# kakaobrain/hqtransformer

Measured on AMD Instinct MI355X. Metric: images/sec (256x256 class-cond sampling), higher is better.
Workload: dtype bf16

## Files before the change

hqtransformer_amd/csrc/common.h:

```cpp
#pragma once
#include <hip/hip_runtime.h>
#include <stdint.h>
#include <string>

typedef uint16_t bf16_t;

__device__ __host__ inline float bf16_to_f32(bf16_t v) {
    union { uint32_t u; float f; } c;
    c.u = ((uint32_t)v) << 16;
    return c.f;
}
__device__ __forceinline__ void bf16x8_to_f32(const uint4& raw, float (&f)[8]) {
    const unsigned w[4] = {raw.x, raw.y, raw.z, raw.w};
#pragma unroll
    for (int i = 0; i < 4; ++i) { f[2 * i] = bf16_to_f32((bf16_t)(w[i] & 0xffffu)); f[2 * i + 1] = bf16_to_f32((bf16_t)(w[i] >> 16)); }
}
__device__ __host__ inline bf16_t f32_to_bf16(float f) {
#if defined(__HIP_DEVICE_COMPILE__)
    return __builtin_bit_cast(bf16_t, (__bf16)f);
#endif
    union { uint32_t u; float f; } c;
    c.f = f;
    if ((c.u & 0x7fffffffu) > 0x7f800000u) return (bf16_t)((c.u >> 16) | 0x40);
    return (bf16_t)((c.u + 0x7fffu + ((c.u >> 16) & 1u)) >> 16);
}

enum { ACT_NONE = 0, ACT_GELU_ERF = 1, ACT_GELU_SIGMOID = 2 };
enum { STORE_ROWS = 0, STORE_NCHW = 1, STORE_QKV = 2, STORE_PACKED = 3, STORE_RESID = 4, STORE_ARGMIN = 5 };

__device__ __host__ inline int conv_ks(int taps) { return taps == 9 ? 3 : (taps == 16 ? 4 : 1); }
__device__ __host__ inline uint32_t float_order_key(float f) {
    union { float f; uint32_t u; } c;
    c.f = f;
    return (c.u & 0x80000000u) ? ~c.u : (c.u | 0x80000000u);
}

__device__ __host__ inline long long packed_off(int m, int k, int MB) {
    return ((long long)(k >> 4) * MB + (m >> 5)) * 512 + ((((k >> 3) & 1) << 5) + (m & 31)) * 8 + (k & 7);
}
constexpr int PACKED_MAX_ROWS = 16384;
__device__ __host__ inline int packed_mb(int M) {
    if (M > PACKED_MAX_ROWS) return 0;
    int mb = 1;
    while (mb * 32 < M) mb <<= 1;
    return mb;
}

struct ChainSync {
    const unsigned* wait;
    unsigned target;
    unsigned* signal;
    unsigned* err;
};

#define HQT_CHAIN_SPIN_LIMIT (1u << 17)
__device__ inline unsigned chain_poll(const ChainSync& c) {
    return c.wait ? __hip_atomic_load(c.wait, __ATOMIC_RELAXED, __HIP_MEMORY_SCOPE_AGENT) : 0u;
}
__device__ inline void chain_wait(const ChainSync& c, unsigned polled) {
    if (!c.wait) return;
    if (threadIdx.x == 0) {
        unsigned spins = 0;
        while (polled < c.target) {
            if (++spins > HQT_CHAIN_SPIN_LIMIT) { if (c.err) *c.err = 1u; break; }
            __builtin_amdgcn_s_sleep(1);
            polled = __hip_atomic_load(c.wait, __ATOMIC_RELAXED, __HIP_MEMORY_SCOPE_AGENT);
        }
        __builtin_amdgcn_fence(__ATOMIC_ACQUIRE, "agent");
        asm volatile("s_waitcnt vmcnt(0)" ::: "memory");
    }
    __syncthreads();
}
__device__ inline void chain_signal(const ChainSync& c) {
    if (!c.signal) return;
    asm volatile("s_waitcnt vmcnt(0)" ::: "memory");
    __syncthreads();
    if (threadIdx.x == 0) {
        __builtin_amdgcn_fence(__ATOMIC_RELEASE, "agent");
        asm volatile("s_waitcnt vmcnt(0)" ::: "memory");
        __hip_atomic_fetch_add(c.signal, 1u, __ATOMIC_RELAXED, __HIP_MEMORY_SCOPE_AGENT);
    }
}

struct GemmArgs {
    const void* A;
    int lda;
    long long a_batch_stride;
    int a_rows_per_group;
    int a_group_stride;
    int a_row_offset;
    int a_packed_mb;
    int conv_taps;
    int conv_stride2;
    int conv_nopad;
    int H, W, Cin;
    int upsample;
    const float* gn_stats;
    const float* gn_gamma;
    const float* gn_beta;
    int gn_groups;
    int gn_swish;
    const void* Bw;
    int ldb;
    long long b_batch_stride;
    void* C;
    int ldc;
    long long c_batch_stride;
    int M, N, K, batch;
    const float* bias;
    const void* resid;
    int act;
    float alpha;
    int store;
    int rows_per_group;
    int group_stride;
    int row_offset;
    const int* row_offset_dev;
    int rows_per_image;
    int clamp01;
    void* C2;
    void* C3;
    int qkv_D;
    int qkv_first;
    bf16_t* qkv_v_pk;
    int c_packed_mb;
    const void* zero_page;
    const float* ln_parts;
    int ln_nparts;
    const float* ln_colsum;
    float ln_eps;
    bf16_t* resid_pk;
    float* resid_parts;
    unsigned* tile_ctr;
    const float* am_rownorm;
    const float* am_colnorm;
    unsigned long long* am_best;
    ChainSync chain;
    float* gn_part_out;
    int gn_out_groups;
    int tune;
    const void* Bw_lo;
    const void* Bw_frag16;
    const void* Bw_up16;
    double* gn_part_out_d;
    int a_f32;
    int b_f32;
    int* range_flag;
    int out_split;
    int k_quarters;
    int b_tile16;
    int k_slices;
    float* k_slabs;
    int tile_panel;
    const int* row_pos;
};

__device__ __forceinline__ int row_live(const int* row_pos, int b) { const int p = row_pos[b]; return p < 0 ? 0 : p; }
__device__ __forceinline__ bool row_idle(const int* row_pos, int b) { return row_pos && row_pos[b] < 0; }
__device__ __forceinline__ int qkv_row_of(const GemmArgs& g, int b, int uniform) { return g.row_pos ? row_live(g.row_pos, b) : uniform; }

struct StepState {
    int step;
    int t_base;
};
__device__ __forceinline__ int step_of(const StepState* state, const int* row_pos, int b) { return row_pos ? row_live(row_pos, b) : state->step; }
struct RowKey {
    unsigned long long seed;
    long long global_row;
};
struct RowSampler {
    float temperature[3];
    int top_k[3];
    float top_p[3];
};
struct GuidePair {
    int pos_row, neg_row;
    float scale[3];
};

#define HQT_MAX_V 16384

__device__ __forceinline__ long long clamp_idx(long long v, int n) { return n > 0 ? (v < 0 ? 0 : (v >= n ? (long long)n - 1 : v)) : v; }
```

hqtransformer_amd/csrc/split_conv.hip:

```cpp
#include "split_kernels.h"
#include "split_ring.h"
#include "gemm_generic.h"
#include <algorithm>
#include <cstdlib>
#include <type_traits>

namespace {
__device__ __forceinline__ unsigned pack_h2(half_t a, half_t b) {
    return (unsigned)__builtin_bit_cast(unsigned short, a) | ((unsigned)__builtin_bit_cast(unsigned short, b) << 16);
}

__device__ __forceinline__ void xcd_tile(int& tile_m, int& tile_n) {
    const int nx = gridDim.x, total = gridDim.x * gridDim.y;
    int id = blockIdx.x + nx * blockIdx.y;
    if ((total & 7) == 0) id = (id & 7) * (total >> 3) + (id >> 3);
    tile_m = id / nx;
    tile_n = id - tile_m * nx;
}
}

__global__ void split_f32_kernel(const float* __restrict__ src, half_t* __restrict__ hi, half_t* __restrict__ lo, size_t n) {
    for (size_t i = blockIdx.x * (size_t)blockDim.x + threadIdx.x; i < n; i += (size_t)gridDim.x * blockDim.x) split2(src[i], hi[i], lo[i]);
}
hipError_t launch_split_f32(const float* src, half_t* hi, half_t* lo, size_t n, hipStream_t st) {
    split_f32_kernel<<<(int)std::min<size_t>((n + 255) / 256, 4096), 256, 0, st>>>(src, hi, lo, n);
    return hipGetLastError();
}

static inline int sp_chunk_pix(int HW) { int c = HW / 32; return c < 64 ? 64 : (c > 1024 ? 1024 : c); }
static inline bool sp_fixed_ok(int C) { return C % 8 == 0 && C / 8 <= 256 && 256 % (C / 8) == 0; }

#ifndef SP_INFLIGHT
#define SP_INFLIGHT 8
#endif
template <bool GN>
__global__ __launch_bounds__(256) void split_pack_kernel(const float* __restrict__ x, half_t* __restrict__ y, const float* __restrict__ stats,
                                                         const float* __restrict__ gamma, const float* __restrict__ beta, int HW, int C, int groups,
                                                         int swish, int nchunk, int chunk_pix, int* __restrict__ range_flag) {
    bool bad = false;
    const int b = blockIdx.x / nchunk, ch = blockIdx.x % nchunk;
    const int p0 = ch * chunk_pix, p1 = min(HW, p0 + chunk_pix);
    const int vpp = C / 8, rpi = 256 / vpp;
    const int cv = threadIdx.x % vpp, pl = threadIdx.x / vpp;
    float mu[8], rs[8], gm[8], bt[8];
    if (GN) {
        const int cpg = C / groups;
#pragma unroll
        for (int i = 0; i < 8; ++i) {
            const int c = cv * 8 + i;
            const float* st = stats + ((long long)b * groups + c / cpg) * 2;
            mu[i] = st[0]; rs[i] = st[1]; gm[i] = gamma[c]; bt[i] = beta[c];
        }
    }
    const float* xb = x + ((long long)b * HW) * C + cv * 8;
    half_t* yb = y + ((long long)b * HW) * 2 * C + cv * 8;
    auto emit = [&](const float4& a0, const float4& a1, int pix) {
        float f[8] = {a0.x, a0.y, a0.z, a0.w, a1.x, a1.y, a1.z, a1.w};
#pragma unroll
        for (int i = 0; i < 8; ++i) {
            if (GN) {
                float t = (f[i] - mu[i]) * rs[i] * gm[i] + bt[i];
                if (swish) t = t * __builtin_amdgcn_rcpf(1.0f + __expf(-t));
                f[i] = t;
            }
        }
        unsigned hi[4], lo[4];
        split8_checked(f, hi, lo, bad);
        const u32x4 vh = {hi[0], hi[1], hi[2], hi[3]};
        const u32x4 vl = {lo[0], lo[1], lo[2], lo[3]};
        half_t* dst = yb + (long long)pix * 2 * C;
        *reinterpret_cast<u32x4*>(dst) = vh;
        *reinterpret_cast<u32x4*>(dst + C) = vl;
    };
    int p = p0 + pl;
    constexpr int UF = SP_INFLIGHT;
    for (; p + (UF - 1) * rpi < p1; p += UF * rpi) {
        float4 r0[UF], r1[UF];
#pragma unroll
        for (int u = 0; u < UF; ++u) {
            const float* s = xb + (long long)(p + u * rpi) * C;
            r0[u] = *reinterpret_cast<const float4*>(s);
            r1[u] = *reinterpret_cast<const float4*>(s + 4);
        }
#pragma unroll
        for (int u = 0; u < UF; ++u) emit(r0[u], r1[u], p + u * rpi);
    }
    for (; p < p1; p += rpi) {
        const float* s = xb + (long long)p * C;
        emit(*reinterpret_cast<const float4*>(s), *reinterpret_cast<const float4*>(s + 4), p);
    }
    if (bad && range_flag) atomicOr(range_flag, 1);
}
__global__ __launch_bounds__(256) void split_pack_generic_kernel(const float* __restrict__ x, half_t* __restrict__ y, const float* __restrict__ stats,
                                                                 const float* __restrict__ gamma, const float* __restrict__ beta, long long total,
                                                                 int HW, int C, int groups, int swish, int* __restrict__ range_flag) {
    const int cpg = stats ? C / groups : 1;
    bool bad = false;
    for (long long i = blockIdx.x * (long long)blockDim.x + threadIdx.x; i < total; i += (long long)gridDim.x * blockDim.x) {
        const long long pix = i / C;
        const int c = (int)(i - pix * C);
        float t = x[i];
        if (stats) {
            const float* st = stats + ((pix / HW) * groups + c / cpg) * 2;
            t = (t - st[0]) * st[1] * gamma[c] + beta[c];
            if (swish) t = t / (1.0f + expf(-t));
        }
        half_t hi, lo;
        split2_checked(t, hi, lo, bad);
        y[pix * 2 * C + c] = hi;
        y[pix * 2 * C + C + c] = lo;
    }
    if (bad && range_flag) atomicOr(range_flag, 1);
}
hipError_t launch_split_pack(const float* x, half_t* y, const float* stats, const float* gamma, const float* beta, int B, int HW,
                             int C, int groups, int swish, int* range_flag, hipStream_t st) {
    if (sp_fixed_ok(C)) {
        const int cp = sp_chunk_pix(HW), nchunk = (HW + cp - 1) / cp;
        if (stats) split_pack_kernel<true><<<B * nchunk, 256, 0, st>>>(x, y, stats, gamma, beta, HW, C, groups, swish, nchunk, cp, range_flag);
        else split_pack_kernel<false><<<B * nchunk, 256, 0, st>>>(x, y, nullptr, nullptr, nullptr, HW, C, groups, 0, nchunk, cp, range_flag);
        return hipGetLastError();
    }
    const long long total = (long long)B * HW * C;
    split_pack_generic_kernel<<<(int)std::min<long long>((total + 255) / 256, 256 * 16), 256, 0, st>>>(x, y, stats, gamma, beta, total, HW, C, groups, swish, range_flag);
    return hipGetLastError();
}

namespace {
constexpr int S_TY = 8, S_TX = 16, S_PITCH = S_TX + 2;
constexpr int S_ROWS = (S_TY + 2) * S_PITCH;
constexpr int S_PIECES = (S_ROWS + 7) / 8;
constexpr int S_PATCH_BYTES = S_PIECES * 1024;
constexpr int S_CPITCH = R_CPITCH;
constexpr int split_conv3_lds(int BN) { return 4 * S_PATCH_BYTES + 4 * BN * 128; }
static_assert(128 * S_CPITCH <= split_conv3_lds(32), "epilogue staging must fit in the operand buffers");
static_assert(split_conv3_lds(128) <= 160 * 1024, "LDS budget");
}

template <bool NCHW, int BN, int PC = 0, int ABL = 0>
__global__ __launch_bounds__(PC ? 512 : 256, 1) void conv3x3_split_kernel(GemmArgs g) {
    static_assert(BN == 128 || (BN == 32 && NCHW), "the 32-channel variant exists for the NCHW conv_out store only");
    constexpr int WMW = BN == 128 ? 2 : 4, FJ = BN == 128 ? 2 : 1, B_BYTES = BN * 128;
    constexpr int FI = (S_TY / 2) / WMW;
    extern __shared__ __attribute__((aligned(16))) char lds_raw[];
    auto PATCH = [&](int s, int plane) -> char* { return lds_raw + (size_t)(s * 2 + plane) * S_PATCH_BYTES; };
    auto BT = [&](int s, int plane) -> char* { return lds_raw + 4 * S_PATCH_BYTES + (size_t)(s * 2 + plane) * B_BYTES; };
    const int tid = threadIdx.x & 255, lane = tid & 63, wave = tid >> 6;
    const bool producer = PC && threadIdx.x >= 256, consumer = !PC || threadIdx.x < 256;
    const int wm = BN == 128 ? wave >> 1 : wave, wn = BN == 128 ? wave & 1 : 0;
    const int fr = lane & 31, fh = lane >> 5;
    int tile_m, tile_n;
    xcd_tile(tile_m, tile_n);
    const int n0 = tile_n * BN;
    const int tiles_x = g.W / S_TX, tiles_y = g.H / S_TY;
    const int img = tile_m / (tiles_x * tiles_y);
    const int trem = tile_m - img * (tiles_x * tiles_y);
    const int ty0 = (trem / tiles_x) * S_TY, tx0 = (trem % tiles_x) * S_TX;
    const int Hin = g.H >> g.upsample, Win = g.W >> g.upsample;
    const half_t* Abase = reinterpret_cast<const half_t*>(g.A);
    const half_t* Bhi = reinterpret_cast<const half_t*>(g.Bw);
    const half_t* Blo = reinterpret_cast<const half_t*>(g.Bw_lo);
    const half_t* zero = reinterpret_cast<const half_t*>(g.zero_page);

    constexpr int PPW = (S_PIECES + 3) / 4;
    constexpr int BPW = BN / 32;
    long long boff[BPW];
#pragma unroll
    for (int i = 0; i < BPW; ++i) {
        const int row = (wave * BPW + i) * 8 + (lane >> 3);
        const int ch = ((lane & 7) ^ ((row >> 1) & 7)) * 8;
        boff[i] = (n0 + row < g.N) ? (long long)(n0 + row) * g.ldb + ch : -1;
    }
    auto issue_patch = [&](int c, int s) {
#pragma unroll
        for (int t = 0; t < PPW; ++t) {
            if (wave + 4 * t < S_PIECES) {
                const int q = (wave + 4 * t) * 8 + (lane >> 3);
                const int qy = (q * 3641) >> 16, qx = q - qy * S_PITCH;
                const int iy = ty0 + qy - 1, ix = tx0 + qx - 1;
                const int ch = ((lane & 7) ^ ((q >> 1) & 7)) * 8;
                const bool in = q < S_ROWS && (unsigned)iy < (unsigned)g.H && (unsigned)ix < (unsigned)g.W;
                const half_t* src = Abase + (((long long)img * Hin + (iy >> g.upsample)) * Win + (ix >> g.upsample)) * (2 * g.Cin) + ch + c * 64;
#pragma unroll
                for (int plane = 0; plane < 2; ++plane) {
                    const half_t* sp = in ? src + plane * g.Cin : zero;
                    char* dst = PATCH(s, plane) + (wave + 4 * t) * 1024;
                    __builtin_amdgcn_global_load_lds((const __attribute__((address_space(1))) void*)sp,
                                                     (__attribute__((address_space(3))) void*)dst, 16, 0, 0);
                }
            }
        }
    };
    auto issue_b = [&](int k0, int s) {
#pragma unroll
        for (int i = 0; i < BPW; ++i) {
            const half_t* sh = boff[i] >= 0 ? Bhi + boff[i] + k0 : zero;
            const half_t* sl = boff[i] >= 0 ? Blo + boff[i] + k0 : zero;
            char* dh = BT(s, 0) + (wave * BPW + i) * 1024;
            char* dl = BT(s, 1) + (wave * BPW + i) * 1024;
            __builtin_amdgcn_global_load_lds((const __attribute__((address_space(1))) void*)sh, (__attribute__((address_space(3))) void*)dh, 16, 0, 0);
            __builtin_amdgcn_global_load_lds((const __attribute__((address_space(1))) void*)sl, (__attribute__((address_space(3))) void*)dl, 16, 0, 0);
        }
    };

    f32x16 accm[FI][FJ], accx[FI][FJ];
#pragma unroll
    for (int i = 0; i < FI; ++i)
#pragma unroll
        for (int j = 0; j < FJ; ++j)
#pragma unroll
            for (int r = 0; r < 16; ++r) { accm[i][j][r] = 0.0f; accx[i][j][r] = 0.0f; }

    int qbase[FI];
#pragma unroll
    for (int i = 0; i < FI; ++i) qbase[i] = (wm * (2 * FI) + i * 2 + (fr >> 4)) * S_PITCH + (fr & 15);
    int brd[FJ];
#pragma unroll
    for (int j = 0; j < FJ; ++j) brd[j] = wn * 64 + j * 32 + fr;

    const unsigned lds_base = (unsigned)(size_t)(__attribute__((address_space(3))) char*)lds_raw;
    unsigned wa0[FJ];
#pragma unroll
    for (int j = 0; j < FJ; ++j) wa0[j] = brd[j] * 128 + ((fh ^ ((brd[j] >> 1) & 7)) << 4);
    auto compute = [&](int ps, int bs, int tapoff) {
        const unsigned pbase = lds_base + ps * 2 * S_PATCH_BYTES, wbase = lds_base + 4 * S_PATCH_BYTES + bs * 2 * B_BYTES;
        unsigned pa0[FI];
#pragma unroll
        for (int i = 0; i < FI; ++i) pa0[i] = (qbase[i] + tapoff) * 128 + ((fh ^ (((qbase[i] + tapoff) >> 1) & 7)) << 4);
        half8 ah[2][FI], al[2][FI], wh[2][FJ], wl[2][FJ];
        auto issue = [&](int ks, int set) {
#pragma unroll
            for (int j = 0; j < FJ; ++j) {
                const unsigned a = wbase + (wa0[j] ^ (ks << 5));
                asm volatile("ds_read_b128 %0, %1" : "=v"(wh[set][j]) : "v"(a));
                asm volatile("ds_read_b128 %0, %1 offset:%2" : "=v"(wl[set][j]) : "v"(a), "n"(B_BYTES));
            }
#pragma unroll
            for (int i = 0; i < FI; ++i) {
                const unsigned a = pbase + (pa0[i] ^ (ks << 5));
                asm volatile("ds_read_b128 %0, %1" : "=v"(ah[set][i]) : "v"(a));
                asm volatile("ds_read_b128 %0, %1 offset:%2" : "=v"(al[set][i]) : "v"(a), "n"(S_PATCH_BYTES));
            }
        };
#define HQT_RETIRE(set, P)                                                                                                          \
// ... 496 lines not shown
```

hqtransformer_amd/csrc/split_device.h:

```cpp
#pragma once
#include "split_kernels.h"

namespace {
constexpr float SPLIT_SCALE = 2048.0f, SPLIT_INV = 1.0f / 2048.0f;

__device__ __forceinline__ void split2(float x, half_t& hi, half_t& lo) {
    hi = (half_t)x;
    lo = (half_t)((x - (float)hi) * SPLIT_SCALE);
}
__device__ __forceinline__ void split2_checked(float x, half_t& hi, half_t& lo, bool& bad) {
    if (!(fabsf(x) < 65504.0f)) { bad = true; x = x > 0.0f ? 65472.0f : (x < 0.0f ? -65472.0f : 0.0f); }
    split2(x, hi, lo);
}
typedef float f32x2_t __attribute__((ext_vector_type(2)));
typedef _Float16 half2_t __attribute__((ext_vector_type(2)));
__device__ __forceinline__ void split8_checked(const float (&x)[8], unsigned (&hi)[4], unsigned (&lo)[4], bool& bad) {
#pragma unroll
    for (int p = 0; p < 4; ++p) {
        f32x2_t v = {x[2 * p], x[2 * p + 1]};
        bad |= !(fabsf(v.x) < 65504.0f) | !(fabsf(v.y) < 65504.0f);
        v.x = __builtin_amdgcn_fmed3f(v.x, -65472.0f, 65472.0f);
        v.y = __builtin_amdgcn_fmed3f(v.y, -65472.0f, 65472.0f);
        const half2_t h = __builtin_convertvector(v, half2_t);
        const f32x2_t r = (v - __builtin_convertvector(h, f32x2_t)) * SPLIT_SCALE;
        const half2_t l = __builtin_convertvector(r, half2_t);
        hi[p] = __builtin_bit_cast(unsigned, h);
        lo[p] = __builtin_bit_cast(unsigned, l);
    }
}
}
```

hqtransformer_amd/csrc/split_stream_conv.hip:

```cpp
#include "split_kernels.h"
#include "split_ring.h"
#include "gemm_generic.h"
#include "switches.h"
#include <algorithm>
#include <cstdlib>
#include <type_traits>

constexpr size_t R_FRAG_PAD = 3 * 4 * 512;
size_t split_frag_elems(int N, int Cin) { return (size_t)((N + 31) / 32) * (Cin / 32) * 9 * 4 * 512 + R_FRAG_PAD; }

__global__ void pack_split_frag16_kernel(const float* __restrict__ w, half_t* __restrict__ out, int N, int Cin, size_t total) {
    const int NC = Cin / 32;
    for (size_t i = blockIdx.x * (size_t)blockDim.x + threadIdx.x; i < total; i += (size_t)gridDim.x * blockDim.x) {
        const int j = (int)(i & 7), lane = (int)((i >> 3) & 63);
        size_t ch = i >> 9;
        const int plane = (int)(ch & 1); ch >>= 1;
        const int blk = (int)(ch & 1); ch >>= 1;
        const int tap = (int)(ch % 9); ch /= 9;
        const int c = (int)(ch % NC);
        const int t = (int)(ch / NC);
        const int n = t * 32 + blk * 16 + (lane & 15), k = tap * Cin + c * 32 + 8 * (lane >> 4) + j;
        const float x = n < N ? w[(size_t)n * 9 * Cin + k] : 0.0f;
        const half_t hi = (half_t)x;
        out[i] = plane ? (half_t)((x - (float)hi) * 2048.0f) : hi;
    }
}
hipError_t launch_pack_split_frag16(const float* w_tapmajor, half_t* out, int N, int Cin, hipStream_t st) {
    const size_t total = split_frag_elems(N, Cin) - R_FRAG_PAD;
    pack_split_frag16_kernel<<<(int)std::min<size_t>((total + 255) / 256, 8192), 256, 0, st>>>(w_tapmajor, out, N, Cin, total);
    return hipGetLastError();
}

namespace {
__device__ __forceinline__ void h_stage_half(char* stage, const f32x4 (&accm)[8][2], const f32x4 (&accx)[8][2], int half, int wave, int fx, int fk) {
#pragma unroll
    for (int ii = 0; ii < 4; ++ii) {
        const int i = half * 4 + ii, r = ii * 16 + fx;
#pragma unroll
        for (int j = 0; j < 2; ++j) {
            const int nl = wave * 32 + j * 16 + 4 * fk;
            f32x4 v;
#pragma unroll
            for (int e = 0; e < 4; ++e) v[e] = accm[i][j][e] + accx[i][j][e] * R_INV;
            *reinterpret_cast<f32x4*>(stage + r * R_CPITCH + nl * 4) = v;
        }
    }
}
}

template <int ABL = 0>
__global__ __launch_bounds__(256, 2) void conv3x3_split_ring16_kernel(GemmArgs g) {
    constexpr int NI = 8;
    extern __shared__ __attribute__((aligned(16))) char lds_raw[];
    const unsigned lds_base = (unsigned)(size_t)(__attribute__((address_space(3))) char*)lds_raw;
    const int tid = threadIdx.x, lane = tid & 63;
    const int wave = __builtin_amdgcn_readfirstlane(tid >> 6);
    const int fx = lane & 15, fk = lane >> 4;
    int tile_m, tile_n;
    r_xcd_tile(tile_m, tile_n, g.tile_panel);
    const int n0 = tile_n * 128;
    int img, trem, ty0, tx0, tiles_x, tiles_y;
    ring_tile(tile_m, g.H, g.W, img, trem, ty0, tx0, tiles_x, tiles_y);
    const int Hin = g.H >> g.upsample, Win = g.W >> g.upsample;
    const int NC = g.Cin / 32;

    const ring_rsrc_t img_rsrc = ring_image_rsrc(g.A, img, Hin, Win, g.Cin);
    unsigned poff[3];
    ring_piece_offsets(poff, wave, lane, ty0, tx0, g.H, g.W, Win, g.upsample, g.Cin);
    u32x4 pst[2];
    unsigned piece_base = ring_piece_base(lds_base, wave, lane);

    const char* bfrag = reinterpret_cast<const char*>(reinterpret_cast<const half_t*>(g.Bw_frag16) + (size_t)(n0 / 32 + wave) * ((size_t)NC * 9 * 2048));
    unsigned lane16 = lane * 16;

    f32x4 accm[NI][2], accx[NI][2];
#pragma unroll
    for (int i = 0; i < NI; ++i)
#pragma unroll
        for (int j = 0; j < 2; ++j)
#pragma unroll
            for (int r = 0; r < 4; ++r) { accm[i][j][r] = 0.0f; accx[i][j][r] = 0.0f; }
    const unsigned abase = ring_frag_base(lds_base, fx, fk);
    half8 ah[4], al[4];
    half8 wh[H_RING][2], wl[H_RING][2];

#pragma unroll
    for (int rnd = 0; rnd < 3; ++rnd) {
        ring_load_piece(pst[0], poff, img_rsrc, 0, 2 * rnd, g.Cin); ring_load_piece(pst[1], poff, img_rsrc, 0, 2 * rnd + 1, g.Cin);
        asm volatile("s_waitcnt vmcnt(0)" : "+v"(pst[0]), "+v"(pst[1]));
        ring_store_piece(piece_base, pst[0], 0, 2 * rnd); ring_store_piece(piece_base, pst[1], 0, 2 * rnd + 1);
    }
#pragma unroll
    for (int s = 0; s < H_AHEAD; ++s) ring_load_b4(wh[s], wl[s], lane16, bfrag, s);
    asm volatile("s_waitcnt vmcnt(0) lgkmcnt(0)" ::: "memory");

#pragma unroll 1
    for (int c0 = 0; c0 < NC; c0 += 2) {
#pragma unroll
        for (int cc = 0; cc < 2; ++cc) {
            const int c = c0 + cc, cn = min(c + 1, NC - 1);
            __builtin_amdgcn_s_barrier();
            __builtin_amdgcn_sched_barrier(0);
            if (ABL != 4) { ring_read_a16(ah, al, abase, cc, 0, 0); ring_read_a16(ah, al, abase, cc, 0, 1); ring_read_a16(ah, al, abase, cc, 0, 2); ring_read_a16(ah, al, abase, cc, 0, 3); }
#pragma unroll
            for (int tap = 0; tap < 9; ++tap) {
                const int s = cc * 9 + tap, slot = s % H_RING, nslot = (s + H_AHEAD) % H_RING;
                const long long S = (long long)c0 * 9 + s;
                const int tapoff = (tap / 3) * R_PITCH + tap % 3, ntapoff = ((tap + 1) / 3) * R_PITCH + (tap + 1) % 3;
                if (ABL != 4) asm volatile("s_waitcnt vmcnt(%4)" : "+v"(wh[slot][0]), "+v"(wl[slot][0]), "+v"(wh[slot][1]), "+v"(wl[slot][1]) : "n"(h_younger(s)));
#pragma unroll
                for (int pr = 0; pr < 4; ++pr) {
                    const int i0 = 2 * pr, i1 = 2 * pr + 1;
                    if (ABL != 4) {
                        const bool more = !(tap == 8 && pr == 3);
                        if (more) asm volatile("s_waitcnt lgkmcnt(4)" : "+v"(ah[i0 % 4]), "+v"(al[i0 % 4]), "+v"(ah[i1 % 4]), "+v"(al[i1 % 4]));
                        else asm volatile("s_waitcnt lgkmcnt(0)" : "+v"(ah[i0 % 4]), "+v"(al[i0 % 4]), "+v"(ah[i1 % 4]), "+v"(al[i1 % 4]));
                    }
#pragma unroll
                    for (int ii = 0; ii < 2; ++ii)
#pragma unroll
                        for (int j = 0; j < 2; ++j)
                            accm[i0 + ii][j] = __builtin_amdgcn_mfma_f32_16x16x32_f16(wh[slot][j], ah[(i0 + ii) % 4], accm[i0 + ii][j], 0, 0, 0);
#pragma unroll
                    for (int ii = 0; ii < 2; ++ii)
#pragma unroll
                        for (int j = 0; j < 2; ++j)
                            accx[i0 + ii][j] = __builtin_amdgcn_mfma_f32_16x16x32_f16(wh[slot][j], al[(i0 + ii) % 4], accx[i0 + ii][j], 0, 0, 0);
#pragma unroll
                    for (int ii = 0; ii < 2; ++ii)
#pragma unroll
                        for (int j = 0; j < 2; ++j)
                            accx[i0 + ii][j] = __builtin_amdgcn_mfma_f32_16x16x32_f16(wl[slot][j], ah[(i0 + ii) % 4], accx[i0 + ii][j], 0, 0, 0);
                    if (ABL == 4) continue;
                    if (pr < 2) {
                        if (pr == 0) { ring_read_a16(ah, al, abase, cc, tapoff, 4); ring_read_a16(ah, al, abase, cc, tapoff, 5); }
                        else { ring_read_a16(ah, al, abase, cc, tapoff, 6); ring_read_a16(ah, al, abase, cc, tapoff, 7); }
                    } else if (tap < 8) {
                        if (pr == 2) { ring_read_a16(ah, al, abase, cc, ntapoff, 0); ring_read_a16(ah, al, abase, cc, ntapoff, 1); }
                        else { ring_read_a16(ah, al, abase, cc, ntapoff, 2); ring_read_a16(ah, al, abase, cc, ntapoff, 3); }
                    }
                    if (pr == 0 && ABL != 5) ring_load_b4(wh[nslot], wl[nslot], lane16, bfrag, S + H_AHEAD);
                    if (pr == 1 && ABL != 2) {
                        if (tap >= 2 && tap - 2 < R_PPW) {
                            if (tap - 1 < R_PPW) asm volatile("s_waitcnt vmcnt(9)" : "+v"(pst[tap % 2]));
                            else asm volatile("s_waitcnt vmcnt(8)" : "+v"(pst[tap % 2]));
                            ring_store_piece(piece_base, pst[tap % 2], cc ^ 1, tap - 2);
                        }
                        if (tap < R_PPW) ring_load_piece(pst[tap % 2], poff, img_rsrc, cn, tap, g.Cin);
                    }
                }
            }
        }
    }
    asm volatile("s_waitcnt vmcnt(0) lgkmcnt(0)" ::: "memory");
    __builtin_amdgcn_s_barrier();
    __builtin_amdgcn_sched_barrier(0);
    if (ABL == 1) { ring_sink_acc(g, accm, accx); return; }
    const long long pix0 = ((long long)img * g.H + ty0) * g.W + tx0;
    char* stage = lds_raw;
    float bv[8], gs[8], gq[8];
    ring_bias8(g, n0 + (tid & 15) * 8, bv);
    bool bad = false;
#pragma unroll
    for (int e = 0; e < 8; ++e) { gs[e] = 0.0f; gq[e] = 0.0f; }
#pragma unroll
    for (int half = 0; half < 2; ++half) {
        if (half > 0) __syncthreads();
        h_stage_half(stage, accm, accx, half, wave, fx, fk);
        __syncthreads();
        ring_store_rows<4, true>(g, stage, tid, n0, bv, true, [&](int r) { return pix0 + (long long)(half * 4 + (r >> 4)) * g.W + (r & 15); }, gs, gq, bad);
    }
    if (bad && g.range_flag) atomicOr(g.range_flag, 1);
    ring_reduce_gn(g, lds_raw, tid, gs, gq, n0, true, (long long)img * (tiles_x * tiles_y) + trem);
}


__global__ void pack_split_up16_kernel(const float* __restrict__ w, half_t* __restrict__ out, int N, int Cin, size_t total) {
    const int NC = Cin / 32, NG = (N + 31) / 32;
    for (size_t i = blockIdx.x * (size_t)blockDim.x + threadIdx.x; i < total; i += (size_t)gridDim.x * blockDim.x) {
        const int j = (int)(i & 7), lane = (int)((i >> 3) & 63);
        size_t ch = i >> 9;
        const int plane = (int)(ch & 1); ch >>= 1;
        const int blk = (int)(ch & 1); ch >>= 1;
        const int tap = (int)(ch & 3); ch >>= 2;
        const int c = (int)(ch % NC); ch /= NC;
        const int t = (int)(ch % NG);
        const int phase = (int)(ch / NG);
        const int pa = phase >> 1, pb = phase & 1, ty = tap >> 1, tx = tap & 1;
        const int n = t * 32 + blk * 16 + (lane & 15), kin = c * 32 + 8 * (lane >> 4) + j;
        const int ky0 = pa == 0 ? (ty == 0 ? 0 : 1) : (ty == 0 ? 0 : 2), ky1 = pa == 0 ? (ty == 0 ? 0 : 2) : (ty == 0 ? 1 : 2);
        const int kx0 = pb == 0 ? (tx == 0 ? 0 : 1) : (tx == 0 ? 0 : 2), kx1 = pb == 0 ? (tx == 0 ? 0 : 2) : (tx == 0 ? 1 : 2);
        double x = 0.0;
        if (n < N)
            for (int ky = ky0; ky <= ky1; ++ky)
                for (int kx = kx0; kx <= kx1; ++kx) x += (double)w[(size_t)n * 9 * Cin + (size_t)(ky * 3 + kx) * Cin + kin];
        const half_t hi = (half_t)(float)x;
        out[i] = plane ? (half_t)(float)((x - (double)(float)hi) * 2048.0) : hi;
    }
}
size_t split_up_elems(int N, int Cin) { return (size_t)4 * ((N + 31) / 32) * (Cin / 32) * 4 * 2048 + 2048; }
hipError_t launch_pack_split_up16(const float* w_tapmajor, half_t* out, int N, int Cin, hipStream_t st) {
    const size_t total = split_up_elems(N, Cin) - 2048;
    pack_split_up16_kernel<<<(int)std::min<size_t>((total + 255) / 256, 8192), 256, 0, st>>>(w_tapmajor, out, N, Cin, total);
    return hipGetLastError();
}

template <int ABL = 0>
__global__ __launch_bounds__(256, 2) void conv2x2_split_up16_kernel(GemmArgs g) {
    constexpr int NI = 8, TAPS = 4;
    extern __shared__ __attribute__((aligned(16))) char lds_raw[];
    const unsigned lds_base = (unsigned)(size_t)(__attribute__((address_space(3))) char*)lds_raw;
    const int tid = threadIdx.x, lane = tid & 63;
    const int wave = __builtin_amdgcn_readfirstlane(tid >> 6);
    const int fx = lane & 15, fk = lane >> 4;
    int tile_m, tile_v;
    r_xcd_tile(tile_m, tile_v, g.tile_panel);
    const int NT = g.N / 128;
    const int phase = tile_v / NT, pa = phase >> 1, pb = phase & 1;
    const int n0 = (tile_v - phase * NT) * 128;
    const int Hin = g.H >> 1, Win = g.W >> 1;
    int img, trem, ty0, tx0, tiles_x, tiles_y;
    ring_tile(tile_m, Hin, Win, img, trem, ty0, tx0, tiles_x, tiles_y);
    const int NC = g.Cin / 32;

    const ring_rsrc_t img_rsrc = ring_image_rsrc(g.A, img, Hin, Win, g.Cin);
    unsigned poff[3];
    ring_piece_offsets(poff, wave, lane, ty0, tx0, Hin, Win, Win, 0, g.Cin);
    u32x4 pst[R_PPW];
    unsigned piece_base = ring_piece_base(lds_base, wave, lane);

    const char* bfrag = reinterpret_cast<const char*>(reinterpret_cast<const half_t*>(g.Bw_up16) +
                                                      ((size_t)phase * (g.N / 32) + n0 / 32 + wave) * ((size_t)NC * TAPS * 2048));
    unsigned lane16 = lane * 16;

    f32x4 accm[NI][2], accx[NI][2];
#pragma unroll
    for (int i = 0; i < NI; ++i)
#pragma unroll
        for (int j = 0; j < 2; ++j)
#pragma unroll
            for (int r = 0; r < 4; ++r) { accm[i][j][r] = 0.0f; accx[i][j][r] = 0.0f; }
    const unsigned abase = ring_frag_base(lds_base, fx + pa * R_PITCH + pb, fk);
    half8 ah[4], al[4];
    half8 wh[2][2], wl[2][2];

#pragma unroll
    for (int u = 0; u < R_PPW; ++u) ring_load_piece(pst[u], poff, img_rsrc, 0, u, g.Cin);
    asm volatile("s_waitcnt vmcnt(0)" : "+v"(pst[0]), "+v"(pst[1]), "+v"(pst[2]), "+v"(pst[3]), "+v"(pst[4]), "+v"(pst[5]));
#pragma unroll
    for (int u = 0; u < R_PPW; ++u) ring_store_piece(piece_base, pst[u], 0, u);
    ring_load_b4(wh[0], wl[0], lane16, bfrag, 0);
    asm volatile("s_waitcnt vmcnt(0) lgkmcnt(0)" ::: "memory");

#pragma unroll 1
    for (int c0 = 0; c0 < NC; c0 += 2) {
#pragma unroll
        for (int cc = 0; cc < 2; ++cc) {
            const int c = c0 + cc, cn = min(c + 1, NC - 1);
            __builtin_amdgcn_s_barrier();
            __builtin_amdgcn_sched_barrier(0);
            if (ABL != 4) { ring_read_a16(ah, al, abase, cc, 0, 0); ring_read_a16(ah, al, abase, cc, 0, 1); ring_read_a16(ah, al, abase, cc, 0, 2); ring_read_a16(ah, al, abase, cc, 0, 3); }
#pragma unroll
            for (int tap = 0; tap < TAPS; ++tap) {
                const int s = cc * TAPS + tap, slot = s % 2, nslot = (s + 1) % 2;
                const long long S = (long long)c0 * TAPS + s;
                const int tapoff = (tap / 2) * R_PITCH + tap % 2, ntapoff = ((tap + 1) / 2) * R_PITCH + (tap + 1) % 2;
                if (ABL != 4) {
                    if (tap == 1 || tap == 2) asm volatile("s_waitcnt vmcnt(3)" : "+v"(wh[slot][0]), "+v"(wl[slot][0]), "+v"(wh[slot][1]), "+v"(wl[slot][1]));
                    else asm volatile("s_waitcnt vmcnt(0)" : "+v"(wh[slot][0]), "+v"(wl[slot][0]), "+v"(wh[slot][1]), "+v"(wl[slot][1]));
                    if (ABL != 5) ring_load_b4(wh[nslot], wl[nslot], lane16, bfrag, S + 1);
                }
#pragma unroll
                for (int pr = 0; pr < 4; ++pr) {
                    const int i0 = 2 * pr, i1 = 2 * pr + 1;
                    if (ABL != 4) {
                        const bool more = !(tap == TAPS - 1 && pr == 3);
                        if (more) asm volatile("s_waitcnt lgkmcnt(4)" : "+v"(ah[i0 % 4]), "+v"(al[i0 % 4]), "+v"(ah[i1 % 4]), "+v"(al[i1 % 4]));
                        else asm volatile("s_waitcnt lgkmcnt(0)" : "+v"(ah[i0 % 4]), "+v"(al[i0 % 4]), "+v"(ah[i1 % 4]), "+v"(al[i1 % 4]));
                    }
#pragma unroll
                    for (int ii = 0; ii < 2; ++ii)
#pragma unroll
                        for (int j = 0; j < 2; ++j)
                            accm[i0 + ii][j] = __builtin_amdgcn_mfma_f32_16x16x32_f16(wh[slot][j], ah[(i0 + ii) % 4], accm[i0 + ii][j], 0, 0, 0);
#pragma unroll
                    for (int ii = 0; ii < 2; ++ii)
#pragma unroll
                        for (int j = 0; j < 2; ++j)
                            accx[i0 + ii][j] = __builtin_amdgcn_mfma_f32_16x16x32_f16(wh[slot][j], al[(i0 + ii) % 4], accx[i0 + ii][j], 0, 0, 0);
#pragma unroll
                    for (int ii = 0; ii < 2; ++ii)
#pragma unroll
                        for (int j = 0; j < 2; ++j)
                            accx[i0 + ii][j] = __builtin_amdgcn_mfma_f32_16x16x32_f16(wl[slot][j], ah[(i0 + ii) % 4], accx[i0 + ii][j], 0, 0, 0);
                    if (ABL == 4) continue;
                    if (pr >= 1 && tap >= 2 && ABL != 2) {
                        const int u = 3 * (tap - 2) + pr - 1;
                        if (tap == 2) asm volatile("s_waitcnt vmcnt(7)" : "+v"(pst[u])); else asm volatile("s_waitcnt vmcnt(4)" : "+v"(pst[u]));
                        ring_store_piece(piece_base, pst[u], cc ^ 1, u);
                    }
                    if (pr < 2) {
                        if (pr == 0) { ring_read_a16(ah, al, abase, cc, tapoff, 4); ring_read_a16(ah, al, abase, cc, tapoff, 5); }
                        else { ring_read_a16(ah, al, abase, cc, tapoff, 6); ring_read_a16(ah, al, abase, cc, tapoff, 7); }
                    } else if (tap < TAPS - 1) {
                        if (pr == 2) { ring_read_a16(ah, al, abase, cc, ntapoff, 0); ring_read_a16(ah, al, abase, cc, ntapoff, 1); }
                        else { ring_read_a16(ah, al, abase, cc, ntapoff, 2); ring_read_a16(ah, al, abase, cc, ntapoff, 3); }
                    }
                    if (pr >= 1 && tap < 2 && ABL != 2) ring_load_piece(pst[3 * tap + pr - 1], poff, img_rsrc, cn, 3 * tap + pr - 1, g.Cin);
                }
            }
        }
    }
    asm volatile("s_waitcnt vmcnt(0) lgkmcnt(0)" ::: "memory");
    __builtin_amdgcn_s_barrier();
    __builtin_amdgcn_sched_barrier(0);
    if (ABL == 1) { ring_sink_acc(g, accm, accx); return; }
    char* stage = lds_raw;
    float bv[8], gs[8], gq[8];
    ring_bias8(g, n0 + (tid & 15) * 8, bv);
#pragma unroll
    for (int e = 0; e < 8; ++e) { gs[e] = 0.0f; gq[e] = 0.0f; }
#pragma unroll
    for (int half = 0; half < 2; ++half) {
        if (half > 0) __syncthreads();
        h_stage_half(stage, accm, accx, half, wave, fx, fk);
        __syncthreads();
        ring_store_rows<4>(g, stage, tid, n0, bv, true, [&](int r) {
            const long long oy = 2 * (ty0 + half * 4 + (r >> 4)) + pa, ox = 2 * (tx0 + (r & 15)) + pb;
            return ((long long)img * g.H + oy) * g.W + ox;
        }, gs, gq);
    }
    ring_reduce_gn(g, lds_raw, tid, gs, gq, n0, true, ((long long)img * (tiles_x * tiles_y) + trem) * 4 + phase);
}


__global__ __launch_bounds__(256, 2) void conv3x3_split_out16_kernel(GemmArgs g) {
    extern __shared__ __attribute__((aligned(16))) char lds_raw[];
    const unsigned lds_base = (unsigned)(size_t)(__attribute__((address_space(3))) char*)lds_raw;
    const int tid = threadIdx.x, lane = tid & 63;
    const int wave = __builtin_amdgcn_readfirstlane(tid >> 6);
    const int fx = lane & 15, fk = lane >> 4;
    const int tile_m = blockIdx.y;
    int img, trem, ty0, tx0, tiles_x, tiles_y;
    ring_tile(tile_m, g.H, g.W, img, trem, ty0, tx0, tiles_x, tiles_y);
    const int Hin = g.H >> g.upsample, Win = g.W >> g.upsample;
    const int NC = g.Cin / 32;

    const ring_rsrc_t img_rsrc = ring_image_rsrc(g.A, img, Hin, Win, g.Cin);
    unsigned poff[3];
    ring_piece_offsets(poff, wave, lane, ty0, tx0, g.H, g.W, Win, g.upsample, g.Cin);
    u32x4 pst[2];
    unsigned piece_base = ring_piece_base(lds_base, wave, lane);

    const char* bfrag = reinterpret_cast<const char*>(g.Bw_frag16);
    unsigned lane16 = lane * 16;

    f32x4 accm[2], accx[2];
#pragma unroll
    for (int i = 0; i < 2; ++i)
#pragma unroll
        for (int r = 0; r < 4; ++r) { accm[i][r] = 0.0f; accx[i][r] = 0.0f; }
    const unsigned abase = ring_frag_base(lds_base, 2 * wave * R_PITCH + fx, fk);
    half8 ah[4], al[4];
    half8 wh[H_RING], wl[H_RING];

#pragma unroll
    for (int rnd = 0; rnd < 3; ++rnd) {
        ring_load_piece(pst[0], poff, img_rsrc, 0, 2 * rnd, g.Cin); ring_load_piece(pst[1], poff, img_rsrc, 0, 2 * rnd + 1, g.Cin);
        asm volatile("s_waitcnt vmcnt(0)" : "+v"(pst[0]), "+v"(pst[1]));
        ring_store_piece(piece_base, pst[0], 0, 2 * rnd); ring_store_piece(piece_base, pst[1], 0, 2 * rnd + 1);
    }
#pragma unroll
    for (int s = 0; s < H_AHEAD; ++s) ring_load_b2(wh[s], wl[s], lane16, bfrag, s);
    asm volatile("s_waitcnt vmcnt(0) lgkmcnt(0)" ::: "memory");

#pragma unroll 1
    for (int c0 = 0; c0 < NC; c0 += 2) {
#pragma unroll
        for (int cc = 0; cc < 2; ++cc) {
            const int c = c0 + cc, cn = min(c + 1, NC - 1);
            __builtin_amdgcn_s_barrier();
            __builtin_amdgcn_sched_barrier(0);
            ring_read_a16(ah, al, abase, cc, 0, 0, 0); ring_read_a16(ah, al, abase, cc, 0, 1, 1);
#pragma unroll
            for (int tap = 0; tap < 9; ++tap) {
                const int s = cc * 9 + tap, slot = s % H_RING, nslot = (s + H_AHEAD) % H_RING;
                const long long S = (long long)c0 * 9 + s;
                const int par = tap & 1;
                const int ntapoff = ((tap + 1) / 3) * R_PITCH + (tap + 1) % 3;
                if (tap < 8) {
                    if (par == 0) { ring_read_a16(ah, al, abase, cc, ntapoff, 0, 2); ring_read_a16(ah, al, abase, cc, ntapoff, 1, 3); }
                    else { ring_read_a16(ah, al, abase, cc, ntapoff, 0, 0); ring_read_a16(ah, al, abase, cc, ntapoff, 1, 1); }
                }
                asm volatile("s_waitcnt vmcnt(%2)" : "+v"(wh[slot]), "+v"(wl[slot]) : "n"(h_younger(s, 2)));
                if (tap < 8) asm volatile("s_waitcnt lgkmcnt(4)" : "+v"(ah[2 * par]), "+v"(al[2 * par]), "+v"(ah[2 * par + 1]), "+v"(al[2 * par + 1]));
                else asm volatile("s_waitcnt lgkmcnt(0)" : "+v"(ah[2 * par]), "+v"(al[2 * par]), "+v"(ah[2 * par + 1]), "+v"(al[2 * par + 1]));
                accm[0] = __builtin_amdgcn_mfma_f32_16x16x32_f16(wh[slot], ah[2 * par], accm[0], 0, 0, 0);
                accm[1] = __builtin_amdgcn_mfma_f32_16x16x32_f16(wh[slot], ah[2 * par + 1], accm[1], 0, 0, 0);
                accx[0] = __builtin_amdgcn_mfma_f32_16x16x32_f16(wh[slot], al[2 * par], accx[0], 0, 0, 0);
                accx[1] = __builtin_amdgcn_mfma_f32_16x16x32_f16(wh[slot], al[2 * par + 1], accx[1], 0, 0, 0);
                accx[0] = __builtin_amdgcn_mfma_f32_16x16x32_f16(wl[slot], ah[2 * par], accx[0], 0, 0, 0);
                accx[1] = __builtin_amdgcn_mfma_f32_16x16x32_f16(wl[slot], ah[2 * par + 1], accx[1], 0, 0, 0);
                ring_load_b2(wh[nslot], wl[nslot], lane16, bfrag, S + H_AHEAD);
                if (tap >= 2 && tap - 2 < R_PPW) {
                    if (tap - 1 < R_PPW) asm volatile("s_waitcnt vmcnt(5)" : "+v"(pst[tap % 2]));
                    else asm volatile("s_waitcnt vmcnt(4)" : "+v"(pst[tap % 2]));
                    ring_store_piece(piece_base, pst[tap % 2], cc ^ 1, tap - 2);
                }
                if (tap < R_PPW) ring_load_piece(pst[tap % 2], poff, img_rsrc, cn, tap, g.Cin);
            }
        }
    }
    asm volatile("s_waitcnt vmcnt(0) lgkmcnt(0)" ::: "memory");
    float* Cb = reinterpret_cast<float*>(g.C);
    const long long hw = (long long)g.H * g.W;
#pragma unroll
    for (int i = 0; i < 2; ++i) {
        const long long pix = (long long)(ty0 + 2 * wave + i) * g.W + tx0 + fx;
#pragma unroll
        for (int r = 0; r < 4; ++r) {
            const int n = 4 * fk + r;
            if (n >= g.N) continue;
            float v = (accm[i][r] + accx[i][r] * R_INV) * g.alpha + (g.bias ? g.bias[n] : 0.0f);
            if (g.clamp01) v = fminf(fmaxf(0.5f * v + 0.5f, 0.0f), 1.0f);
            Cb[((long long)img * g.N + n) * hw + pix] = v;
        }
    }
}

bool split_conv3_emits_planes(const GemmArgs& g) {
    const bool off = !switch_value(SW_SPLIT_PLANES_OUT);
    return !off && split_stream_ok(g) && g.store == STORE_ROWS && !g.upsample && g.ldc == g.N && g.N % 8 == 0;
}
bool split_stream_ok(const GemmArgs& g) {
    if (!g.Bw_frag16) return false;
    if (g.H % R_TY != 0 || g.W % R_TX != 0 || g.Cin % 64 != 0) return false;
    if ((long long)(g.H >> g.upsample) * (g.W >> g.upsample) * g.Cin * 4 >= (1ll << 31)) return false;
    if (g.store == STORE_NCHW) return g.N <= 16;
    return g.N % 128 == 0 && g.ldc % 8 == 0;
}
static bool split_up_shape(const GemmArgs& g) {
    const bool off = !switch_value(SW_SPLIT_UP);
    return !off && g.upsample == 1 && g.Bw_up16 && g.store == STORE_ROWS && (g.H / 2) % R_TY == 0 && (g.W / 2) % R_TX == 0 && g.N % 128 == 0;
}
int split_stream_tiles_per_image(const GemmArgs& g) { return split_up_shape(g) ? 4 * (g.H / 2 / R_TY) * (g.W / 2 / R_TX) : (g.H / R_TY) * (g.W / R_TX); }
hipError_t launch_split_conv3_stream(const GemmArgs& g, hipStream_t st) {
    if (g.store == STORE_NCHW) conv3x3_split_out16_kernel<<<dim3(1, g.M / (R_TY * R_TX), 1), 256, G_LDS, st>>>(g);
    else if (split_up_shape(g)) conv2x2_split_up16_kernel<0><<<dim3(4 * (g.N / 128), g.M / 4 / (R_TY * R_TX), 1), 256, G_LDS, st>>>(g);
    else conv3x3_split_ring16_kernel<0><<<dim3(g.N / 128, g.M / (R_TY * R_TX), 1), 256, G_LDS, st>>>(g);
    return hipGetLastError();
}
hipError_t split_stream_configure() {
    hipError_t e = hipFuncSetAttribute(reinterpret_cast<const void*>(conv3x3_split_ring16_kernel<0>), hipFuncAttributeMaxDynamicSharedMemorySize, G_LDS);
    if (e != hipSuccess) return e;
    e = hipFuncSetAttribute(reinterpret_cast<const void*>(conv2x2_split_up16_kernel<0>), hipFuncAttributeMaxDynamicSharedMemorySize, G_LDS);
    if (e != hipSuccess) return e;
    return hipFuncSetAttribute(reinterpret_cast<const void*>(conv3x3_split_out16_kernel), hipFuncAttributeMaxDynamicSharedMemorySize, G_LDS);
}

namespace {
constexpr int O_T = 16, O_P = O_T + 2, O_CH = 32, O_PITCH = O_CH + 4;
constexpr int O_LDS = O_P * O_P * O_PITCH * 4;
constexpr int O_V4 = O_P * O_P * (O_CH / 4);
constexpr int O_PER = (O_V4 + 255) / 256;
typedef __attribute__((ext_vector_type(2))) float f32x2;
}

template <int NO>
__global__ __launch_bounds__(256, 3) void conv_out_direct_kernel(GemmArgs g) {
    extern __shared__ __attribute__((aligned(16))) char lds_raw[];
    float* patch = reinterpret_cast<float*>(lds_raw);
    const int tid = threadIdx.x;
    const int tiles_x = g.W / O_T, tiles = tiles_x * (g.H / O_T);
    const int img = blockIdx.x / tiles, trem = blockIdx.x - img * tiles;
    const int ty0 = (trem / tiles_x) * O_T, tx0 = (trem % tiles_x) * O_T;
    const int C = g.Cin, NC = C / O_CH;
    const float* __restrict__ X = reinterpret_cast<const float*>(g.A) + (long long)img * g.H * g.W * C;
    const float* __restrict__ Wt = reinterpret_cast<const float*>(g.Bw);
    const int v = tid & 7;
    int src[O_PER];
    unsigned inside = 0;
#pragma unroll
    for (int u = 0; u < O_PER; ++u) {
        const int q = (tid + 256 * u) >> 3;
        const int qy = q / O_P, qx = q - qy * O_P;
// ... 91 lines not shown
```

Baseline: 1666.

## Piggyback split-pack work onto conv kernels via a rider descriptor

Moves the split-pack loop into a reusable device function and adds a SplitRider descriptor to GemmArgs. Conv kernels can then execute a slice of an independent split-pack job, either before or after their main tile work, to avoid a separate kernel launch. This adds register pressure and work imbalance to the conv kernels. No host code enabling the rider is present yet.

Result: slower. 1641 (-1.5%).

```diff
diff --git a/hqtransformer_amd/csrc/common.h b/hqtransformer_amd/csrc/common.h
--- a/hqtransformer_amd/csrc/common.h
+++ b/hqtransformer_amd/csrc/common.h
@@ -2,6 +2,7 @@
 #include <hip/hip_runtime.h>
 #include <stdint.h>
 #include <string>
+#include "split_rider.h"
 
 typedef uint16_t bf16_t;
 
@@ -153,6 +154,7 @@
     float* k_slabs;
     int tile_panel;
     const int* row_pos;
+    SplitRider rider;
 };
 
 __device__ __forceinline__ int row_live(const int* row_pos, int b) { const int p = row_pos[b]; return p < 0 ? 0 : p; }
diff --git a/hqtransformer_amd/csrc/split_conv.hip b/hqtransformer_amd/csrc/split_conv.hip
--- a/hqtransformer_amd/csrc/split_conv.hip
+++ b/hqtransformer_amd/csrc/split_conv.hip
@@ -28,11 +28,6 @@
 }
 
 static inline int sp_chunk_pix(int HW) { int c = HW / 32; return c < 64 ? 64 : (c > 1024 ? 1024 : c); }
-static inline bool sp_fixed_ok(int C) { return C % 8 == 0 && C / 8 <= 256 && 256 % (C / 8) == 0; }
-
-#ifndef SP_INFLIGHT
-#define SP_INFLIGHT 8
-#endif
 template <bool GN>
 __global__ __launch_bounds__(256) void split_pack_kernel(const float* __restrict__ x, half_t* __restrict__ y, const float* __restrict__ stats,
                                                          const float* __restrict__ gamma, const float* __restrict__ beta, int HW, int C, int groups,
@@ -40,55 +35,7 @@
     bool bad = false;
     const int b = blockIdx.x / nchunk, ch = blockIdx.x % nchunk;
     const int p0 = ch * chunk_pix, p1 = min(HW, p0 + chunk_pix);
-    const int vpp = C / 8, rpi = 256 / vpp;
-    const int cv = threadIdx.x % vpp, pl = threadIdx.x / vpp;
-    float mu[8], rs[8], gm[8], bt[8];
-    if (GN) {
-        const int cpg = C / groups;
-#pragma unroll
-        for (int i = 0; i < 8; ++i) {
-            const int c = cv * 8 + i;
-            const float* st = stats + ((long long)b * groups + c / cpg) * 2;
-            mu[i] = st[0]; rs[i] = st[1]; gm[i] = gamma[c]; bt[i] = beta[c];
-        }
-    }
-    const float* xb = x + ((long long)b * HW) * C + cv * 8;
-    half_t* yb = y + ((long long)b * HW) * 2 * C + cv * 8;
-    auto emit = [&](const float4& a0, const float4& a1, int pix) {
-        float f[8] = {a0.x, a0.y, a0.z, a0.w, a1.x, a1.y, a1.z, a1.w};
-#pragma unroll
-        for (int i = 0; i < 8; ++i) {
-            if (GN) {
-                float t = (f[i] - mu[i]) * rs[i] * gm[i] + bt[i];
-                if (swish) t = t * __builtin_amdgcn_rcpf(1.0f + __expf(-t));
-                f[i] = t;
-            }
-        }
-        unsigned hi[4], lo[4];
-        split8_checked(f, hi, lo, bad);
-        const u32x4 vh = {hi[0], hi[1], hi[2], hi[3]};
-        const u32x4 vl = {lo[0], lo[1], lo[2], lo[3]};
-        half_t* dst = yb + (long long)pix * 2 * C;
-        *reinterpret_cast<u32x4*>(dst) = vh;
-        *reinterpret_cast<u32x4*>(dst + C) = vl;
-    };
-    int p = p0 + pl;
-    constexpr int UF = SP_INFLIGHT;
-    for (; p + (UF - 1) * rpi < p1; p += UF * rpi) {
-        float4 r0[UF], r1[UF];
-#pragma unroll
-        for (int u = 0; u < UF; ++u) {
-            const float* s = xb + (long long)(p + u * rpi) * C;
-            r0[u] = *reinterpret_cast<const float4*>(s);
-            r1[u] = *reinterpret_cast<const float4*>(s + 4);
-        }
-#pragma unroll
-        for (int u = 0; u < UF; ++u) emit(r0[u], r1[u], p + u * rpi);
-    }
-    for (; p < p1; p += rpi) {
-        const float* s = xb + (long long)p * C;
-        emit(*reinterpret_cast<const float4*>(s), *reinterpret_cast<const float4*>(s + 4), p);
-    }
+    split_pack_run<GN>(x, y, stats, gamma, beta, HW, C, groups, swish, threadIdx.x, b, p0, p1, bad);
     if (bad && range_flag) atomicOr(range_flag, 1);
 }
 __global__ __launch_bounds__(256) void split_pack_generic_kernel(const float* __restrict__ x, half_t* __restrict__ y, const float* __restrict__ stats,
diff --git a/hqtransformer_amd/csrc/split_device.h b/hqtransformer_amd/csrc/split_device.h
--- a/hqtransformer_amd/csrc/split_device.h
+++ b/hqtransformer_amd/csrc/split_device.h
@@ -28,4 +28,78 @@
         lo[p] = __builtin_bit_cast(unsigned, l);
     }
 }
+
+#ifndef SP_INFLIGHT
+#define SP_INFLIGHT 8
+#endif
+typedef __attribute__((ext_vector_type(4))) unsigned int u32x4;
+template <bool GN>
+__device__ __forceinline__ void split_pack_run(const float* __restrict__ x, half_t* __restrict__ y, const float* __restrict__ stats,
+                                               const float* __restrict__ gamma, const float* __restrict__ beta, int HW, int C, int groups, int swish,
+                                               int tid, int b, int p0, int p1, bool& bad) {
+    const int vpp = C / 8, rpi = 256 / vpp;
+    const int cv = tid % vpp, pl = tid / vpp;
+    float mu[8], rs[8], gm[8], bt[8];
+    if (GN) {
+        const int cpg = C / groups;
+#pragma unroll
+        for (int i = 0; i < 8; ++i) {
+            const int c = cv * 8 + i;
+            const float* st = stats + ((long long)b * groups + c / cpg) * 2;
+            mu[i] = st[0]; rs[i] = st[1]; gm[i] = gamma[c]; bt[i] = beta[c];
+        }
+    }
+    const float* xb = x + ((long long)b * HW) * C + cv * 8;
+    half_t* yb = y + ((long long)b * HW) * 2 * C + cv * 8;
+    auto emit = [&](const float4& a0, const float4& a1, int pix) {
+        float f[8] = {a0.x, a0.y, a0.z, a0.w, a1.x, a1.y, a1.z, a1.w};
+#pragma unroll
+        for (int i = 0; i < 8; ++i) {
+            if (GN) {
+                float t = (f[i] - mu[i]) * rs[i] * gm[i] + bt[i];
+                if (swish) t = t * __builtin_amdgcn_rcpf(1.0f + __expf(-t));
+                f[i] = t;
+            }
+        }
+        unsigned hi[4], lo[4];
+        split8_checked(f, hi, lo, bad);
+        const u32x4 vh = {hi[0], hi[1], hi[2], hi[3]};
+        const u32x4 vl = {lo[0], lo[1], lo[2], lo[3]};
+        half_t* dst = yb + (long long)pix * 2 * C;
+        *reinterpret_cast<u32x4*>(dst) = vh;
+        *reinterpret_cast<u32x4*>(dst + C) = vl;
+    };
+    int p = p0 + pl;
+    constexpr int UF = SP_INFLIGHT;
+    for (; p + (UF - 1) * rpi < p1; p += UF * rpi) {
+        float4 r0[UF], r1[UF];
+#pragma unroll
+        for (int u = 0; u < UF; ++u) {
+            const float* s = xb + (long long)(p + u * rpi) * C;
+            r0[u] = *reinterpret_cast<const float4*>(s);
+            r1[u] = *reinterpret_cast<const float4*>(s + 4);
+        }
+#pragma unroll
+        for (int u = 0; u < UF; ++u) emit(r0[u], r1[u], p + u * rpi);
+    }
+    for (; p < p1; p += rpi) {
+        const float* s = xb + (long long)p * C;
+        emit(*reinterpret_cast<const float4*>(s), *reinterpret_cast<const float4*>(s + 4), p);
+    }
 }
+
+__device__ __forceinline__ void split_rider_run(const SplitRider& r, int wg, int nwg, int tid) {
+    long long q, q1;
+    sp_rider_slice(wg, nwg, (long long)r.images * r.HW, 256 / (r.C / 8), q, q1);
+    bool bad = false;
+    half_t* y = reinterpret_cast<half_t*>(r.y);
+    while (q < q1) {
+        const int b = (int)(q / r.HW);
+        const int p0 = (int)(q - (long long)b * r.HW), p1 = (int)(q1 - (long long)b * r.HW < r.HW ? q1 - (long long)b * r.HW : r.HW);
+        if (r.stats) split_pack_run<true>(r.x, y, r.stats, r.gamma, r.beta, r.HW, r.C, r.groups, r.swish, tid, b, p0, p1, bad);
+        else split_pack_run<false>(r.x, y, nullptr, nullptr, nullptr, r.HW, r.C, r.groups, 0, tid, b, p0, p1, bad);
+        q += p1 - p0;
+    }
+    if (bad && r.range_flag) atomicOr(r.range_flag, 1);
+}
+}
diff --git a/hqtransformer_amd/csrc/split_rider.h b/hqtransformer_amd/csrc/split_rider.h
--- /dev/null
+++ b/hqtransformer_amd/csrc/split_rider.h
@@ -0,0 +1,26 @@
+#pragma once
+
+#if defined(__HIPCC__) || defined(__CUDACC__)
+#define SPLIT_RIDER_HD __host__ __device__
+#else
+#define SPLIT_RIDER_HD
+#endif
+
+struct SplitRider {
+    const float* x;
+    void* y;
+    const float* stats;
+    const float* gamma;
+    const float* beta;
+    int* range_flag;
+    int images, HW, C, groups, swish;
+};
+
+SPLIT_RIDER_HD inline bool sp_fixed_ok(int C) { return C % 8 == 0 && C / 8 <= 256 && 256 % (C / 8) == 0; }
+
+SPLIT_RIDER_HD inline void sp_rider_slice(long long wg, long long nwg, long long total, int gran, long long& p0, long long& p1) {
+    long long per = (total + nwg - 1) / nwg;
+    per = (per + gran - 1) / gran * gran;
+    p0 = wg * per < total ? wg * per : total;
+    p1 = p0 + per < total ? p0 + per : total;
+}
diff --git a/hqtransformer_amd/csrc/split_stream_conv.hip b/hqtransformer_amd/csrc/split_stream_conv.hip
--- a/hqtransformer_amd/csrc/split_stream_conv.hip
+++ b/hqtransformer_amd/csrc/split_stream_conv.hip
@@ -63,6 +63,7 @@
     ring_tile(tile_m, g.H, g.W, img, trem, ty0, tx0, tiles_x, tiles_y);
     const int Hin = g.H >> g.upsample, Win = g.W >> g.upsample;
     const int NC = g.Cin / 32;
+    if (ABL == 6 && g.rider.x) split_rider_run(g.rider, tile_m * (int)gridDim.x + tile_n, (int)(gridDim.x * gridDim.y), tid);
 
     const ring_rsrc_t img_rsrc = ring_image_rsrc(g.A, img, Hin, Win, g.Cin);
     unsigned poff[3];
@@ -172,6 +173,7 @@
     }
     if (bad && g.range_flag) atomicOr(g.range_flag, 1);
     ring_reduce_gn(g, lds_raw, tid, gs, gq, n0, true, (long long)img * (tiles_x * tiles_y) + trem);
+    if (ABL != 6 && g.rider.x) split_rider_run(g.rider, tile_m * (int)gridDim.x + tile_n, (int)(gridDim.x * gridDim.y), tid);
 }
 
 
@@ -222,6 +224,7 @@
     int img, trem, ty0, tx0, tiles_x, tiles_y;
     ring_tile(tile_m, Hin, Win, img, trem, ty0, tx0, tiles_x, tiles_y);
     const int NC = g.Cin / 32;
+    if (ABL == 6 && g.rider.x) split_rider_run(g.rider, tile_m * (int)gridDim.x + tile_v, (int)(gridDim.x * gridDim.y), tid);
 
     const ring_rsrc_t img_rsrc = ring_image_rsrc(g.A, img, Hin, Win, g.Cin);
     unsigned poff[3];
@@ -331,6 +334,7 @@
         }, gs, gq);
     }
     ring_reduce_gn(g, lds_raw, tid, gs, gq, n0, true, ((long long)img * (tiles_x * tiles_y) + trem) * 4 + phase);
+    if (ABL != 6 && g.rider.x) split_rider_run(g.rider, tile_m * (int)gridDim.x + tile_v, (int)(gridDim.x * gridDim.y), tid);
 }
 
 
```
